# jkomijani/normflow_

Hardware: AMD Instinct MI355X
Metric: lattice configs/sec (forward+logdet) (higher is better)
Workload: dtype f32

## Files before the change

### normflow__amd/_hip.py

```python
import ctypes as C
import os
import threading
import weakref

import torch

_HERE = os.path.dirname(os.path.abspath(__file__))
LIB_PATH = os.path.join(_HERE, "lib", "libnormflow_hip.so")

NF_F32, NF_F64, NF_F16, NF_F16_FIELD = 0, 1, 2, 3
LAYOUT_FULL, LAYOUT_PAIR = 0, 1
EXTRAP = {None: 0, 'none': 0, 'linear': 1, 'anti': 2, 'anti-periodic': 2}


OPT_SPLIT16, OPT_PIPE, OPT_SMALL8 = 0, 1, 2


class NormflowHipError(RuntimeError):
    pass


class RqsOpts(C.Structure):
    _fields_ = [("m", C.c_int32), ("extrap_left", C.c_int32), ("extrap_right", C.c_int32),
                ("layout", C.c_int32), ("xlo", C.c_double), ("xhi", C.c_double),
# ... 528 lines not shown
    return wp.reshape(nt, 16, cin_pad // 4, 4, ntaps).permute(4, 2, 0, 3, 1).contiguous()


def conv_weight_for_layer(w, lat4, k4, cin, cout, compact, fused, dtype_code):
    frag = pack_conv_weight(w)
    code = load().nf_conv_weight_layout(lat4, k4, cin, cout, int(compact), int(fused), dtype_code)
    if code < 0:
        raise RuntimeError("nf_conv_weight_layout: invalid layer description")
    if code == 0:
        return frag
    if code == 2:
        return pack_conv_weight_split16(w)
    ntaps, kq, nt = frag.shape[:3]
    k3 = w.shape[-1]
    rows = ntaps // k3
    vals = frag.reshape(rows, k3, kq, nt, 64).permute(0, 2, 4, 1, 3).reshape(rows, kq, 64, k3 * nt)
    nv = (k3 * nt + 3) // 4 * 4
    out = vals.new_zeros(rows, kq, 64, nv)
    out[..., :k3 * nt] = vals
    return out.contiguous()


SPLIT16_WEIGHT_SCALE = 1024.0


def pack_conv_weight_split16(w):
    cout, cin = w.shape[:2]
    assert cin == 8 and tuple(w.shape[2:]) == (3, 3, 3, 3) and cout <= 48
    wp = w.new_zeros(48, 8, 28, 3, dtype=torch.float32)
    wp[:cout, :, :27] = w.reshape(cout, 8, 27, 3).float() * SPLIT16_WEIGHT_SCALE
    hi = wp.half()
    lo = (wp - hi.float()).half()
    out = torch.empty(3, 21, 2, 64, 8, dtype=torch.float16, device=w.device)
    for k, part in enumerate((hi, lo)):
        v = part.reshape(3, 16, 8, 7, 4, 3).permute(0, 5, 3, 4, 1, 2)
        out[:, :, k] = v.reshape(3, 21, 64, 8)
    return out.contiguous()


def pack_conv_weight_split16_two_site(w):
    assert tuple(w.shape) == (8, 8, 3, 3, 3, 3)
    wr = w.reshape(8, 8, 27, 3).float() * SPLIT16_WEIGHT_SCALE
    w2 = wr.new_zeros(16, 8, 27, 4)
    w2[:8, :, :, :3] = wr
    w2[8:, :, :, 1:] = wr
    hi = w2.half()
    lo = (w2 - hi.float()).half()
    out = torch.empty(27, 2, 64, 8, dtype=torch.float16, device=w.device)
    for k, part in enumerate((hi, lo)):
        out[:, k] = part.permute(2, 3, 0, 1).reshape(27, 64, 8)
    return out.contiguous()


def pack_conv_weight_split16_first(w):
    assert tuple(w.shape) == (8, 1, 3, 3, 3, 3)
    wr = w.reshape(8, 27, 3).float() * SPLIT16_WEIGHT_SCALE
    w2 = wr.new_zeros(16, 32, 4)
    w2[:8, :27, :3] = wr
    w2[8:, :27, 1:] = wr
    hi = w2.half()
    lo = (w2 - hi.float()).half()
    out = torch.empty(4, 2, 64, 8, dtype=torch.float16, device=w.device)
    for k, part in enumerate((hi, lo)):
        v = part.reshape(16, 4, 4, 2, 4).permute(1, 2, 0, 3, 4)
        out[:, k] = v.reshape(4, 64, 8)
    return out.contiguous()


def conv_first_split16(x, weight, bias, act, weight_src=None):
    lib = load()
    B = x.shape[0]
    lat = list(x.shape[2:])
    lat4 = (C.c_int32 * 4)(*lat)
    V = 1
    for n in lat:
        V *= n
    wsp = _cached_pack(weight if weight_src is None else weight_src, 'first16', pack_conv_weight_split16_first)
    bias = None if bias is None else bias.detach().float().contiguous()
    out = torch.empty((B, V, 16), dtype=torch.float16, device=x.device)
    step = max(1, min(MAX_B, ((1 << 31) - 1) // V))
    for b0 in range(0, B, step):
        b1 = min(B, b0 + step)
        _check(lib.nf_conv_first_split16(_ptr(x[b0:b1]), _ptr(wsp), _ptr(bias), _ptr(out[b0:b1]), b1 - b0, lat4,
                                         int(act), _stream()), "nf_conv_first_split16")
    return out


def _split16_site_index(L3, device):
    slot = torch.arange(L3 // 2, device=device)
    return torch.stack((2 * slot, (2 * slot - 1) % L3))


def to_split16(h):
    B, Cc = h.shape[:2]
    L3 = h.shape[-1]
    if Cc != 8 or L3 % 2:
        raise NormflowHipError("to_split16: 8 channels and an even fastest axis expected")
    hp = h.reshape(B, 8, -1, L3).float()
    idx = _split16_site_index(L3, h.device)
    g = hp[..., idx].permute(0, 2, 3, 4, 1)
    hi = g.half()
    lo = (g - hi.float()).half()
    return torch.stack((hi, lo), dim=2).reshape(B, -1, 16).contiguous()


def from_split16(h16, lattice):
    B = h16.shape[0]
    L3 = lattice[-1]
    t = h16.reshape(B, -1, 2, 2, L3 // 2, 8).float()
    v = t[:, :, 0] + t[:, :, 1]
    idx = _split16_site_index(L3, h16.device)
    out = torch.empty((B, v.shape[1], L3, 8), dtype=torch.float32, device=h16.device)
    out[:, :, idx.reshape(-1)] = v.reshape(B, v.shape[1], L3, 8)
    return out.permute(0, 3, 1, 2).reshape((B, 8) + tuple(lattice)).contiguous()


def conv_layer_split16(h16, weight, bias, act, lattice):
    lib = load()
    B = h16.shape[0]
    lat4 = (C.c_int32 * 4)(*lattice)
    wsp = _cached_pack(weight, 'two_site16', pack_conv_weight_split16_two_site)
    bias = None if bias is None else bias.detach().float().contiguous()
    out = torch.empty_like(h16)
    for b0 in range(0, B, MAX_B):
        b1 = min(B, b0 + MAX_B)
        _check(lib.nf_conv_fwd_split16(_ptr(h16[b0:b1]), _ptr(wsp), _ptr(bias), _ptr(out[b0:b1]), b1 - b0, lat4,
                                       int(act), _stream()), "nf_conv_fwd_split16")
    return out


_UNIT_OK = {}


def invalidate_weight_checks():
    _UNIT_OK.clear()
    _PACKED.clear()


_PACKED = {}
_PACK_IN_CAPTURE = [False]


class pack_inside_capture:

    def __enter__(self):
        self._old = _PACK_IN_CAPTURE[0]
        _PACK_IN_CAPTURE[0] = True

    def __exit__(self, *exc):
        _PACK_IN_CAPTURE[0] = self._old
        return False


def _cached_pack(w, kind, fn):
    if _PACK_IN_CAPTURE[0] and torch.cuda.is_current_stream_capturing():
        return fn(w.detach())
    base = w._base if w._base is not None else w
    key = (id(base), kind)
    state = (w._version, w.data_ptr(), tuple(w.shape), w.dtype)
    hit = _PACKED.get(key)
    if hit is not None and hit[0]() is base and hit[1] == state:
        return hit[2]
    out = fn(w.detach())
    _PACKED[key] = (weakref.ref(base, lambda _, k=key: _PACKED.pop(k, None)), state, out)
    return out


def _weights_fit_fp16(w):
    base = w._base if w._base is not None else w
    key = id(base)
    state = (w._version, w.data_ptr(), tuple(w.shape))
    hit = _UNIT_OK.get(key)
    if hit is not None and hit[0]() is base and hit[1] == state:
        return hit[2]
# ... 120 lines not shown
            if split:
                need = lib.nf_conv_wgrad_split16_workspace(b1 - b0, lat4, cin)
                ws = torch.empty(int(need), dtype=torch.uint8, device=x.device)
                if bits is None:
                    bits = absmax_bits(gz)
                _check(lib.nf_conv_wgrad_split16(_ptr(x[b0:b1]), _ptr(part[b0:b1]), _ptr(buf), b1 - b0, lat4, k4, cin,
                                                 c1 - c0, _ptr(bits), int(compact_parity), _ptr(ws), ws.numel(), _stream()),
                       "nf_conv_wgrad_split16")
            elif sites:
                need = lib.nf_conv_wgrad_sites_workspace(k4, cin, c1 - c0, _dtype_code(x))
                ws = torch.empty(int(need), dtype=torch.uint8, device=x.device)
                _check(lib.nf_conv_wgrad_sites(_ptr(x[b0:b1]), _ptr(part[b0:b1]), _ptr(buf), b1 - b0, lat4, k4, cin,
                                               c1 - c0, int(compact_parity), _ptr(ws), ws.numel(), _dtype_code(x), _stream()),
                       "nf_conv_wgrad_sites")
            else:
                _check(lib.nf_conv_wgrad(_ptr(x[b0:b1]), _ptr(part[b0:b1]), _ptr(buf), b1 - b0, lat4, k4, cin,
                                         c1 - c0, _dtype_code(x), _stream()), "nf_conv_wgrad")
        gws.append(buf[:c1 - c0, :ntaps * cin])
        gbs.append(buf[:c1 - c0, ntaps * cin])
    gw = torch.cat(gws) if len(gws) > 1 else gws[0]
    gb = torch.cat(gbs) if len(gbs) > 1 else gbs[0]
    gw = gw.reshape(cout, ntaps, cin).permute(0, 2, 1).reshape((cout, cin) + tuple(ksize))
    return gw, gb


def conv_input_grad_split16(gz, wt, bits=None, compact_parity=-1, lattice=None, weight=None):
    lib = load()
    cin = wt.shape[0]
    if compact_parity < 0:
        lattice = tuple(gz.shape[2:])
    if (gz.dtype != torch.float32 or lattice is None or len(lattice) != 4 or cin > 8 or tuple(wt.shape[2:]) != (3, 3, 3, 3)
            or not lib.nf_get_option(OPT_SPLIT16)):
        return None
    B, Cc = gz.shape[:2]
    lat4, k4 = _lat4(lattice, (3, 3, 3, 3))
    if not lib.nf_conv_split16_supported(lat4, k4, 8, 8, ACT_CODES['tanh']) or B > 65535:
        return None
    if not _weights_fit_fp16(wt if weight is None else weight):
        return None
    G = (Cc + 7) // 8
    V = 1
    for n in lattice:
        V *= n
    gz = gz.contiguous()
    g16 = torch.empty((G, B, V, 16), dtype=torch.float16, device=gz.device)
    if bits is None:
        bits = absmax_bits(gz)
    _check(lib.nf_planes_to_split16(_ptr(gz), _ptr(g16), _ptr(bits), B, Cc, lat4, int(compact_parity), _stream()),
           "nf_planes_to_split16")
    gx = torch.empty((B, 8) + tuple(lattice), dtype=torch.float32, device=gz.device)
    wpad = wt.new_zeros((8, 8 * G, 3, 3, 3, 3), dtype=torch.float32)
    wpad[:cin, :Cc] = wt.float()
    for g in range(G):
        wsp = pack_conv_weight_split16_two_site(wpad[:, 8 * g:8 * g + 8].contiguous())
        _check(lib.nf_conv_dgrad_split16(_ptr(g16[g]), _ptr(wsp), None, _ptr(gx), B, lat4, _ptr(bits), int(g > 0), 0,
                                         _stream()), "nf_conv_dgrad_split16")
    return gx if cin == 8 else gx[:, :cin].contiguous()


def conv_hidden_planes_split16(x, weight, bias, act):
    lib = load()
    if (x.dtype != torch.float32 or x.dim() != 6 or tuple(weight.shape) != (8, 8, 3, 3, 3, 3) or act not in (0, ACT_CODES['tanh'])
            or not lib.nf_get_option(OPT_SPLIT16)):
        return None
    B = x.shape[0]
    lattice = tuple(x.shape[2:])
    lat4, k4 = _lat4(lattice, (3, 3, 3, 3))
    if not lib.nf_conv_split16_supported(lat4, k4, 8, 8, ACT_CODES['tanh']) or B > 65535 or not _weights_fit_fp16(weight):
        return None
    V = x[0, 0].numel()
    x16 = torch.empty((1, B, V, 16), dtype=torch.float16, device=x.device)
    bits = absmax_bits(x)
    _check(lib.nf_planes_to_split16(_ptr(x), _ptr(x16), _ptr(bits), B, 8, lat4, -1, _stream()), "nf_planes_to_split16")
    wsp = pack_conv_weight_split16_two_site(weight.detach().float())
    out = torch.empty_like(x)
    b = None if bias is None else bias.detach().float().contiguous()
    _check(lib.nf_conv_dgrad_split16(_ptr(x16[0]), _ptr(wsp), _ptr(b), _ptr(out), B, lat4, _ptr(bits), 0, int(act), _stream()),
           "nf_conv_dgrad_split16")
    return out


def conv_last_logits_split16(x, weight, bias, parity):
    lib = load()
    if (x.dtype != torch.float32 or x.dim() != 6 or tuple(weight.shape) != (46, 8, 3, 3, 3, 3) or x.shape[1] != 8
            or x.shape[-1] < 32 or x.shape[-1] % 16 or any(n < 2 or n % 2 for n in x.shape[2:5])
            or not lib.nf_get_option(OPT_SPLIT16) or not _weights_fit_fp16(weight)):
        return None
    B = x.shape[0]
    lattice = tuple(x.shape[2:])
    lat4 = (C.c_int32 * 4)(*lattice)
    V = x[0, 0].numel()
    bits = absmax_bits(x)
    wsp = pack_conv_weight_split16(weight.detach().float())
    b = None if bias is None else bias.detach().float().contiguous()
    out = torch.empty((B, 46, V // 2), dtype=torch.float32, device=x.device)
    src, is16 = x, 0
    if lattice[-1] != 32:
        src = torch.empty((1, B, V, 16), dtype=torch.float16, device=x.device)
        _check(lib.nf_planes_to_split16(_ptr(x), _ptr(src), _ptr(bits), B, 8, lat4, -1, _stream()), "nf_planes_to_split16")
        is16 = 1
    _check(lib.nf_conv_last_logits_split16(_ptr(src), is16, _ptr(wsp), _ptr(b), _ptr(out), B, lat4, int(parity), _ptr(bits),
                                           _stream()), "nf_conv_last_logits_split16")
    return out


def pack_wide_split16(w1, b1, w2, b2, w3, b3):
    h, cout = w1.shape[0], w3.shape[0]
    f = lambda t: t.detach().float()
    w1p = f(w1).new_zeros((16, 1, 3, 3, 3, 3)); w1p[:h] = f(w1)
    w2p = f(w2).new_zeros((16, 16, 3, 3, 3, 3)); w2p[:h, :h] = f(w2)
    w3p = f(w3).new_zeros((cout, 16, 3, 3, 3, 3)); w3p[:, :h] = f(w3)
    padb = lambda b, n: None if b is None else torch.nn.functional.pad(f(b), (0, n - b.shape[0]))
    b1p, b2p = padb(b1, 16), padb(b2, 16)
    cut = lambda b, g: None if b is None else b[8 * g:8 * g + 8].contiguous()
    first = [(pack_conv_weight_split16_first(w1p[8 * g:8 * g + 8].contiguous()), cut(b1p, g)) for g in (0, 1)]
    hidden = [[pack_conv_weight_split16_two_site(w2p[8 * go:8 * go + 8, 8 * gi:8 * gi + 8].contiguous()) for gi in (0, 1)] for go in (0, 1)]
    last = [pack_conv_weight_split16(w3p[:, 8 * gi:8 * gi + 8].contiguous()) for gi in (0, 1)]
    return first, (hidden, [cut(b2p, 0), cut(b2p, 1)]), (last, None if b3 is None else f(b3).contiguous()), cout


def conv_wide_logits_split16(x, packed, act1, parity):
    lib = load()
    first, (hidden, hb), (last, b3), cout = packed
    B = x.shape[0]
    lattice = tuple(x.shape[2:])
    lat4 = (C.c_int32 * 4)(*lattice)
    V = x[0, 0].numel()
    x = x.contiguous()
    tanh = ACT_CODES['tanh']
    h1 = []
    for wsp, b in first:
        out = torch.empty((B, V, 16), dtype=torch.float16, device=x.device)
        _check(lib.nf_conv_first_split16(_ptr(x), _ptr(wsp), _ptr(b), _ptr(out), B, lat4, int(act1), _stream()), "nf_conv_first_split16")
        h1.append(out)
    h2 = []
    z = torch.empty((B, 8) + lattice, dtype=torch.float32, device=x.device)
    for go in (0, 1):
        for gi in (0, 1):
            _check(lib.nf_conv_dgrad_split16(_ptr(h1[gi]), _ptr(hidden[go][gi]), _ptr(hb[go]) if gi == 0 else None, _ptr(z), B, lat4, None,
                                             int(gi > 0), tanh if gi == 1 else 0, _stream()), "nf_conv_dgrad_split16")
        out = torch.empty((1, B, V, 16), dtype=torch.float16, device=x.device)
        _check(lib.nf_planes_to_split16(_ptr(z), _ptr(out), None, B, 8, lat4, -1, _stream()), "nf_planes_to_split16")
        h2.append(out)
    del h1
    logits = torch.empty((B, cout, V // 2), dtype=torch.float32, device=x.device)
    for gi in (0, 1):
        _check(lib.nf_conv_last_logits_split16_acc(_ptr(h2[gi]), 1, _ptr(last[gi]), _ptr(b3) if gi == 0 else None, _ptr(logits), B, lat4,
                                                   int(parity), None, int(gi > 0), int(cout), _stream()), "nf_conv_last_logits_split16_acc")
    return logits


class ConvFn(torch.autograd.Function):

    @staticmethod
    def forward(ctx, x, weight, bias, act, compact, parity):
        _require_device(x, weight, bias)
        x = x.contiguous()
        out = None
        if not compact and x.dim() == 6 and x.shape[1] == 8 and weight.shape[0] == 8:
            out = conv_hidden_planes_split16(x, weight, bias, act)
        elif compact and act == 0 and x.dim() == 6 and weight.shape[0] == 46:
            out = conv_last_logits_split16(x, weight, bias, parity)
        if out is None:
            out = _conv_launch(x, weight.detach(), bias, act, compact, parity, weight_src=weight)
        ctx.save_for_backward(x, weight, out if act else None)
        ctx.act, ctx.compact, ctx.parity, ctx.has_bias = act, compact, parity, bias is not None
        return out

    @staticmethod
# ... 81 lines not shown
        return y, logj

    @staticmethod
    def backward(ctx, gy, glogj):
        h, weight, bias, xpt = ctx.saved_tensors
        lib = load()
        B, V = xpt.shape
        lattice = tuple(h.shape[2:])
        lat4 = (C.c_int32 * 4)(*lattice)
        cout = weight.shape[0]
        bits = absmax_bits(h)
        src, is16 = FusedLastRqsFn._source(h, bits, lat4)
        wsp = pack_conv_weight_split16(weight.detach().float())
        b = None if bias is None else bias.detach().float().contiguous()
        gz = torch.empty((B, cout, V // 2), dtype=torch.float32, device=h.device)
        gx = torch.empty_like(xpt)
        _check(lib.nf_conv_rqs_split16_vjp(_ptr(src), is16, _ptr(wsp), _ptr(b), cout, _ptr(xpt), _ptr(gy.contiguous()),
                                           _ptr(glogj.contiguous()), _ptr(gz), _ptr(gx), B, lat4, int(ctx.parity), _ptr(bits),
                                           C.byref(ctx.opts), int(bool(ctx.inverse)), _stream()), "nf_conv_rqs_split16_vjp")
        gh = gw = gb = None
        gbits = absmax_bits(gz)
        if ctx.needs_input_grad[0]:
            wt = weight.detach().flip([2, 3, 4, 5]).transpose(0, 1).contiguous()
            gh = conv_input_grad_split16(gz, wt, gbits, ctx.parity, lattice, weight)
        if ctx.needs_input_grad[1] or (bias is not None and ctx.needs_input_grad[2]):
            got = conv_weight_grad(h, gz, weight.shape[2:], gbits, ctx.parity)
            if got is not None:
                gw, gb = got
        if (ctx.needs_input_grad[0] and gh is None) or ((ctx.needs_input_grad[1] or ctx.needs_input_grad[2]) and gw is None):
            raise NormflowHipError("FusedLastRqsFn.backward: the split-fp16 gradient kernels refused a layer the forward pass took")
        if bias is None:
            gb = None
        return gh, gw, gb, gx, (glogj if ctx.has_log0 else None), None, None, None


def conv_layer(x, weight, bias, act=0, compact=False, parity=0):
    if torch.is_grad_enabled() and (x.requires_grad or weight.requires_grad or (bias is not None and bias.requires_grad)):
        if act == 5:
            return torch.abs(ConvFn.apply(x, weight, bias, 0, compact, parity))
        return ConvFn.apply(x, weight, bias, act, compact, parity)
    x = x.contiguous()
    return _conv_launch(x, weight.detach(), None if bias is None else bias.detach(), act, compact, parity, weight_src=weight)


def conv_affine_split16(h16, weight, bias, x_active, log0, parity, inverse, lattice, out=None):
    _require_device(h16, weight, bias, x_active, log0)
    lib = load()
    B, V = x_active.shape
    x_active = x_active.contiguous()
    lat4 = (C.c_int32 * 4)(*lattice)
    def pack_affine(w):
        w8 = w.new_zeros((8, 8, 3, 3, 3, 3), dtype=torch.float32)
        w8[:2] = w.float()
        return pack_conv_weight_split16_two_site(w8)
    wsp = _cached_pack(weight, 'affine16', pack_affine)
    b8 = torch.zeros(8, dtype=torch.float32, device=x_active.device)
    if bias is not None:
        b8[:2] = bias.detach().float()
    field16 = x_active.dtype == torch.float16
    if out is None:
        y = torch.empty_like(x_active)
        logj = torch.empty(B, dtype=torch.float32, device=x_active.device)
    else:
        y, logj = out
    ws = _workspace(min(B, MAX_B), V, x_active.device)
    for b0 in range(0, B, MAX_B):
        b1 = min(B, b0 + MAX_B)
        l0 = log0[b0:b1] if log0 is not None else None
        _check(lib.nf_conv_affine_split16(_ptr(h16[b0:b1]), _ptr(wsp), _ptr(b8), _ptr(x_active[b0:b1]), _ptr(l0),
                                          _ptr(y[b0:b1]), _ptr(logj[b0:b1]), b1 - b0, lat4, int(parity), int(inverse),
                                          4 if field16 else 0, _ptr(ws), ws.numel(), _stream()), "nf_conv_affine_split16")
    return y, logj


def conv_rqs(h, weight, bias, x_active, log0, parity, opts, inverse, unit_input=False, lattice=None, out=None):
    _require_device(h, weight, bias, x_active, log0)
    lib = load()
    h, x_active = h.contiguous(), x_active.contiguous()
    split_in = lattice is not None
    B = h.shape[0]
    cin = weight.shape[1] if split_in else h.shape[1]
    lat = list(lattice) if split_in else list(h.shape[2:])
    d = len(lat)
    lat4 = (C.c_int32 * 4)(*([1] * (4 - d) + lat))
    k4 = (C.c_int32 * 4)(*([1] * (4 - d) + list(weight.shape[2:])))
    V = x_active.shape[1]
    flags = 1 if (unit_input and _weights_fit_fp16(weight)) else 0
    field16 = x_active.dtype == torch.float16
    if field16:
        flags |= 4
    ldt = torch.float32 if field16 else x_active.dtype
    if split_in:
        if not flags or h.dtype != torch.float16 or tuple(h.shape) != (B, V, 16):
            raise NormflowHipError("split-fp16 hidden activations need unit_input and a (B, V, 16) half tensor")
        flags |= 2
    fused_code = 1 | ((flags & 1) << 1) | ((flags & 2) << 1)
    kind = ('fused_last', tuple(lat4), tuple(k4), cin, fused_code, lib.nf_get_option(OPT_SPLIT16), lib.nf_get_option(OPT_PIPE))
    wfrag = _cached_pack(weight, kind, lambda w: conv_weight_for_layer(w, lat4, k4, cin, w.shape[0], True, fused_code, NF_F32))
    bias = None if bias is None else bias.detach().contiguous()
    if out is None:
        y = torch.empty_like(x_active)
        logj = torch.empty(B, dtype=ldt, device=x_active.device)
    else:
        y, logj = out
        if (tuple(y.shape) != (B, V) or tuple(logj.shape) != (B,) or y.dtype != x_active.dtype or logj.dtype != ldt
                or not y.is_contiguous() or not logj.is_contiguous()):
            raise NormflowHipError("conv_rqs: `out` must be contiguous (B, V) and (B,) tensors of the input's dtype (log|J| fp32 for a half field)")
        _require_device(y, logj)
# ... 157 lines not shown
```

### normflow__amd/csrc/nf_conv_g.hip

```cpp
#include <hip/hip_runtime.h>
#include <hip/hip_fp16.h>
#include "nf_conv_core.h"

namespace nf {

typedef _Float16 f16x8 __attribute__((ext_vector_type(8)));
typedef _Float16 f16x4 __attribute__((ext_vector_type(4)));

#if !defined(NF_DIAG) || !defined(NF_G2_ABL)
#undef NF_G2_ABL
#define NF_G2_ABL 0
#endif

namespace g2 {
template <bool SEGM>
struct Geo {
  static constexpr int RBL = SEGM ? 1088 : 1024;
  static constexpr int PLROWS = 16;
  static constexpr int PLANE = PLROWS * RBL;
  static constexpr int NSLOT = 8;
  static constexpr int RING = NSLOT * PLANE;
  static constexpr int XBUF = 4 * 2 * 64 * 16;
  static constexpr int LDS_BYTES = RING + 2 * XBUF;
  static_assert(LDS_BYTES <= 160 * 1024, "ring + exchange must fit the CU's LDS");
};
#ifndef NF_G2_PRIO
#define NF_G2_PRIO 1
#endif
constexpr int NSA = 14;
constexpr float kInvWScale = 1.0f / 1024.0f;
}

__device__ __forceinline__ float tanh_affine(float a, float c1, float c0) {
  const float t = __builtin_amdgcn_exp2f(__builtin_fmaf(a, c1, c0));
  return __builtin_fmaf(-2.0f, __builtin_amdgcn_rcpf(1.0f + t), 1.0f);
}
__device__ __forceinline__ float act_affine(float a, float c1, float c0, float al, float ga) {
  const float t = __builtin_amdgcn_exp2f(__builtin_fmaf(a, c1, c0));
  return __builtin_fmaf(al, __builtin_amdgcn_rcpf(1.0f + t), ga);
}

template <bool SEGM, int EPI, bool HK = false>
__global__ __launch_bounds__(512, 2) void conv_g2_kernel(ConvArgs A) {
  using namespace g2;
  typedef Geo<SEGM> G;
  constexpr int RBL = G::RBL, PLANE = G::PLANE, NSLOT = G::NSLOT, RING = G::RING, XBUF = G::XBUF;
  extern __shared__ __align__(16) unsigned char smem_g2[];
  const int lane = threadIdx.x & 63;
  const int wave = __builtin_amdgcn_readfirstlane(threadIdx.x >> 6);
  const bool isB = wave >= 4;
  const int q = wave & 3;
  const int g = lane >> 4, p = lane & 15;
  const unsigned lds0 = unsigned(reinterpret_cast<size_t>((__attribute__((address_space(3))) unsigned char *)smem_g2));

  const int n0 = A.L[0] >> 1, n1 = A.L[1] >> 1, ncol = n0 * n1;
  const int L2 = A.L[2], nstep = L2 >> 1;
  const int L3 = A.L[3], HP = L3 >> 1, NSEG = (HP + 15) >> 4;
  const int RB = L3 * 32, HB = L3 * 16, PB = L3 * 8;
  const int seg_lo = SEGM ? A.seg_lo : 0, seg_n = SEGM ? (A.seg_n > 0 ? A.seg_n : NSEG) : 1;
  const int total = int(A.nitems);
  const int xcd = blockIdx.x & 7, jm = blockIdx.x >> 3;
  auto col_id = [&](int ci) { return (xcd + 8 * ci) * 32 + jm; };
  int ncols_my = 0;
  {
    const int first = col_id(0);
    if (first < total) ncols_my = (total - first + 255) / 256;
  }
  if (ncols_my == 0) return;
  const int td0 = NSEG == 1 ? 1 : ((n0 & 3) == 0 ? 4 : ((n0 & 1) == 0 ? 2 : 1));
  const int td1 = NSEG == 1 ? 1 : ((n1 & 3) == 0 ? 4 : ((n1 & 1) == 0 ? 2 : 1));
  auto decode = [&](int ci, int &b, int &i0, int &i1, int &hs) {
    int gc = col_id(ci);
    hs = 0;
    if (SEGM) {
      hs = seg_lo + gc % seg_n;
      gc /= seg_n;
    }
    b = gc / ncol;
    int c = gc - b * ncol;
    const int t1 = c % td1; c /= td1;
    const int t0 = c % td0; c /= td0;
    const int nt1 = n1 / td1;
    i0 = (c / nt1) * td0 + t0;
    i1 = (c % nt1) * td1 + t1;
  };

  const int sl0 = isB ? NSA : 0;
  f16x8 bh[NSA], bl[NSA];
  {
    const f16x8 *__restrict__ wsp = static_cast<const f16x8 *>(A.wfrag) + lane;
#pragma unroll
    for (int r = 0; r < NSA; ++r) {
      const int rr = sl0 + r;
      const int rc = rr < 27 ? rr : 26;
      bh[r] = wsp[(2 * rc) * 64];
      bl[r] = wsp[(2 * rc + 1) * 64];
    }
  }
  float bv4[4], kc0[4];
#pragma unroll
  for (int r = 0; r < 4; ++r) {
    bv4[r] = A.bias ? static_cast<const float *>(A.bias)[4 * (g & 1) + r] : 0.f;
  }
  const bool is_tanh = A.act != kActSigmoid;
  const float kcs = is_tanh ? 2.885390081777927f : -1.4426950408889634f;
  const float kal = is_tanh ? -2.0f : 1.0f, kga = is_tanh ? 1.0f : 0.0f;
#pragma unroll
  for (int r = 0; r < 4; ++r) kc0[r] = kcs * bv4[r];
  const float kc1 = kcs * kInvWScale;
  [[maybe_unused]] const float descale = kInvWScale / pow2_scale_for(A.gscale_bits);

  const int ja = p + (g >> 1), para = (g + 1) & 1;
  const unsigned rowsel = unsigned(((q >> 1) * 4 + (q & 1)) * RBL);
  const unsigned lane_a = rowsel + unsigned((SEGM && ja == 16) ? 1024 + para * 16 : para * 256 + (ja & 15) * 16);
  const unsigned lane_al = lane_a + unsigned((SEGM && ja == 16) ? 32 : 512);
  constexpr bool HALF = SEGM && EPI != 3 && HK;
  const int psh = p >> 3, pm = p & 7;
  const int lane_am_delta = int(rowsel + unsigned(para * 256 + (pm + (g >> 1)) * 16)) - int(lane_a);
  const int hz0 = wave >> 1, hz1a = 2 * (wave & 1);
  unsigned lane_d = unsigned(lane * 16), lane_d2 = 0;
  const unsigned char *__restrict__ inb = static_cast<const unsigned char *>(A.in);
  const int64_t sampleB = A.V * 32;

  int ici = 0, ipl = -1, head = 0;
  const unsigned char *rowp[2] = {nullptr, nullptr};
  auto open_issue_column = [&]() {
    int ib, ii0, ii1, hs;
    decode(ici, ib, ii0, ii1, hs);
    int x0 = 2 * ii0 + hz0 - 1;
    x0 = x0 < 0 ? x0 + A.L[0] : (x0 >= A.L[0] ? x0 - A.L[0] : x0);
#pragma unroll
    for (int k = 0; k < 2; ++k) {
      int x1 = 2 * ii1 + hz1a + k - 1;
      x1 = x1 < 0 ? x1 + A.L[1] : (x1 >= A.L[1] ? x1 - A.L[1] : x1);
      rowp[k] = inb + int64_t(ib) * sampleB + int64_t((x0 * A.L[1] + x1) * L2) * RB;
    }
    if (SEGM) {
      const int blk = lane >> 4;
      int gs = 16 * hs + (lane & 15);
      gs = gs >= HP ? gs - HP : gs;
      lane_d = unsigned((blk >> 1) * HB + (blk & 1) * PB + gs * 16);
      int g17 = 16 * hs + 16;
      g17 = g17 >= HP ? g17 - HP : g17;
      lane_d2 = unsigned(((lane >> 1) & 1) * HB + (lane & 1) * PB + g17 * 16);
    }
  };
  open_issue_column();
  const unsigned lds_rows = lds0 + unsigned((hz0 * 4 + hz1a) * RBL);
  constexpr int PPP = SEGM ? 2 : 1;
  auto issue_piece = [&](int k) {
    if (ici >= ncols_my) return false;
    const int x2 = ipl < 0 ? L2 - 1 : (ipl >= L2 ? 0 : ipl);
    const unsigned char *src = rowp[k] + unsigned(x2) * unsigned(RB);
    const unsigned dst = lds_rows + unsigned((head & (NSLOT - 1)) * PLANE + k * RBL);
    dma_row(src, lane_d, dst);
    if (SEGM) {
      if (lane < 4) dma_row(src, lane_d2, dst + 1024u);
    }
    if (k == 1) {
      ++head;
      if (++ipl > L2) {
        ipl = -1;
        if (++ici < ncols_my) open_issue_column();
      }
    }
    return true;
  };
  auto issue_entry = [&]() { return issue_piece(0) && issue_piece(1); };

#pragma unroll 1
  for (int e = 0; e < NSLOT; ++e) (void)issue_entry();
// ... 80 lines not shown
        hi[r] = h0;
        lo[r] = static_cast<_Float16>(v - static_cast<float>(h0));
      }
      if (plane_ok) {
        unsigned char *d = pout + plane_o;
        *reinterpret_cast<f16x4 *>(d) = hi;
        *reinterpret_cast<f16x4 *>(d + HB) = lo;
      }
    } else if constexpr (EPI == 3) {
      if (plane_ok) {
        float *d = static_cast<float *>(A.out) + pfield + int64_t(4 * (g & 1)) * A.V;
#pragma unroll
        for (int r = 0; r < 4; ++r) {
          float v = (prev[r] + pa[r]) * descale + bv4[r];
          if (A.accumulate) v += pold[r];
          if (A.act == kActTanh) v = tanh_affine(v, 2.885390081777927f, 0.f);
          d[int64_t(r) * A.V] = v;
        }
      }
    } else {
      if (pslot != aslot) {
        flush();
        aslot = pslot;
      }
      if (plane_ok) {
        const float t = (prev[0] + pa[0]) * kInvWScale + bv4[0];
        const float sa = __builtin_fabsf((prev[1] + pa[1]) * kInvWScale + bv4[1]);
        const float2 xv = load_field_pair(A, pfield);
        const int a = g >> 1;
        const float v = a ? xv.y : xv.x;
        const float val = EPI == 2 ? (v - t) * nf_exp(sa) : t + v * nf_exp(-sa);
        float2 ov;
        ov.x = a ? 0.f : val;
        ov.y = a ? val : 0.f;
        store_field_pair(A, pfield, ov);
        lacc += double(EPI == 2 ? sa : -sa);
      }
    }
  };

  for (int k = 0; k < nsteps_total; ++k) {
    int ndma = 0;
    if (EPI == 3 && A.accumulate) {
      if (lane_ok) {
        const float *d = static_cast<const float *>(A.out) + fcol + int64_t(2 * s) * L3 + int64_t(4 * (g & 1)) * A.V;
#pragma unroll
        for (int r = 0; r < 4; ++r) nold[r] = d[int64_t(r) * A.V];
      }
    }
    if (!(NF_G2_ABL & 1) && free_next == 4) {
      ndma += issue_entry() ? 2 * PPP : 0;
      ndma += issue_entry() ? 2 * PPP : 0;
    }
    const bool refill = !(NF_G2_ABL & 1) && free_next >= 2;
    auto dma_slot = [&](int i) {
      if (refill && issue_piece(i & 1)) ndma += PPP;
    };
    NF_G2TICK(0)
    if (isB && have_prev && !(NF_G2_ABL & 2)) epilogue((k - 1) & 1);
    NF_G2TICK(1)
#if NF_G2_PRIO
    __builtin_amdgcn_s_setprio(2);
#endif
    f32x4 am[2], ac[2];
    am[0] = am[1] = ac[0] = ac[1] = f32x4{0.f, 0.f, 0.f, 0.f};
    unsigned rowa[4], rowl[4];
#pragma unroll
    for (int i = 0; i < 4; ++i) {
      const unsigned po = unsigned(((rbase + i) & (NSLOT - 1)) * PLANE);
      rowa[i] = po + lane_a;
      rowl[i] = po + lane_al;
    }
    auto fetch = [&](f16x8 (&fh)[4], f16x8 (&fl)[4], int coff, int I0, int I1, int H0, int H1) {
      if constexpr (HALF) {
#pragma unroll
        for (int i = 0; i < 3; ++i) {
          if (i < H0 || i > H1) continue;
          const unsigned rm = unsigned(((rbase + i + psh) & (NSLOT - 1)) * PLANE) + unsigned(int(lane_a) + lane_am_delta);
          fh[i] = *reinterpret_cast<const f16x8 *>(smem_g2 + rm + coff);
          fl[i] = *reinterpret_cast<const f16x8 *>(smem_g2 + rm + 512 + coff);
        }
        return;
      }
#pragma unroll
      for (int i = 0; i < 4; ++i) {
        if (i < I0 || i > I1) continue;
        if (NF_G2_ABL & 8) {
          fh[i] = bh[i]; fl[i] = bl[i];
          asm volatile("" : "+v"(fh[i]), "+v"(fl[i]));
        } else {
          fh[i] = *reinterpret_cast<const f16x8 *>(smem_g2 + rowa[i] + coff);
          fl[i] = *reinterpret_cast<const f16x8 *>(smem_g2 + rowl[i] + coff);
        }
      }
    };
    auto mult = [&](const f16x8 (&fh)[4], const f16x8 (&fl)[4], int base, int J0, int J1) {
      if (NF_G2_ABL & 4) {
#pragma unroll
        for (int i = 0; i < 4; ++i) asm volatile("" ::"v"(fh[i]), "v"(fl[i]));
        return;
      }
      if constexpr (HALF) {
#pragma unroll
        for (int j2 = 0; j2 < 3; ++j2)
          if (j2 >= J0 && j2 <= J1) am[0] = __builtin_amdgcn_mfma_f32_16x16x32_f16(bh[base + j2], fh[j2], am[0], 0, 0, 0);
#pragma unroll
        for (int j2 = 0; j2 < 3; ++j2)
          if (j2 >= J0 && j2 <= J1) ac[0] = __builtin_amdgcn_mfma_f32_16x16x32_f16(bl[base + j2], fh[j2], ac[0], 0, 0, 0);
#pragma unroll
        for (int j2 = 0; j2 < 3; ++j2)
          if (j2 >= J0 && j2 <= J1) ac[0] = __builtin_amdgcn_mfma_f32_16x16x32_f16(bh[base + j2], fl[j2], ac[0], 0, 0, 0);
        return;
      }
#pragma unroll
      for (int j2 = 0; j2 < 3; ++j2)
#pragma unroll
        for (int t = 0; t < 2; ++t)
          if (j2 >= J0 && j2 <= J1) am[t] = __builtin_amdgcn_mfma_f32_16x16x32_f16(bh[base + j2], fh[t + j2], am[t], 0, 0, 0);
#pragma unroll
      for (int j2 = 0; j2 < 3; ++j2)
#pragma unroll
        for (int t = 0; t < 2; ++t)
          if (j2 >= J0 && j2 <= J1) ac[t] = __builtin_amdgcn_mfma_f32_16x16x32_f16(bl[base + j2], fh[t + j2], ac[t], 0, 0, 0);
#pragma unroll
      for (int j2 = 0; j2 < 3; ++j2)
#pragma unroll
        for (int t = 0; t < 2; ++t)
          if (j2 >= J0 && j2 <= J1) ac[t] = __builtin_amdgcn_mfma_f32_16x16x32_f16(bh[base + j2], fl[t + j2], ac[t], 0, 0, 0);
    };
    auto combo_off = [](int jj) { return ((jj / 3) * 4 + jj % 3) * RBL; };
    f16x8 fh0[4], fl0[4], fh1[4], fl1[4];
#define NF_SB __builtin_amdgcn_sched_barrier(0)
    if (!isB) {
      fetch(fh0, fl0, combo_off(0), 0, 3, 0, 2);
      fetch(fh1, fl1, combo_off(1), 0, 3, 0, 2);
      NF_SB; mult(fh0, fl0, 0, 0, 2); NF_SB;
      dma_slot(0);
      fetch(fh0, fl0, combo_off(2), 0, 3, 0, 2);
      NF_SB; mult(fh1, fl1, 3, 0, 2); NF_SB;
      dma_slot(1);
      fetch(fh1, fl1, combo_off(3), 0, 3, 0, 2);
      NF_SB; mult(fh0, fl0, 6, 0, 2); NF_SB;
      dma_slot(2);
      fetch(fh0, fl0, combo_off(4), 0, 2, 0, 1);
      NF_SB; mult(fh1, fl1, 9, 0, 2); NF_SB;
      dma_slot(3);
      mult(fh0, fl0, 12, 0, 1);
      NF_SB;
    } else {
      fetch(fh0, fl0, combo_off(4), 2, 3, 2, 2);
      fetch(fh1, fl1, combo_off(5), 0, 3, 0, 2);
      NF_SB; mult(fh0, fl0, 12 - NSA, 2, 2); NF_SB;
      fetch(fh0, fl0, combo_off(6), 0, 3, 0, 2);
      NF_SB; mult(fh1, fl1, 15 - NSA, 0, 2); NF_SB;
      dma_slot(0);
      fetch(fh1, fl1, combo_off(7), 0, 3, 0, 2);
      NF_SB; mult(fh0, fl0, 18 - NSA, 0, 2); NF_SB;
      dma_slot(1);
      fetch(fh0, fl0, combo_off(8), 0, 3, 0, 2);
      NF_SB; mult(fh1, fl1, 21 - NSA, 0, 2); NF_SB;
      dma_slot(2);
      mult(fh0, fl0, 24 - NSA, 0, 2);
      NF_SB;
      dma_slot(3);
    }
#undef NF_SB
#if NF_G2_PRIO
    __builtin_amdgcn_s_setprio(0);
#endif
    if (!isB && have_prev && !(NF_G2_ABL & 2)) epilogue((k - 1) & 1);
    NF_G2TICK(2)
#pragma unroll
    for (int t = 0; t < 2; ++t)
#pragma unroll
      for (int r = 0; r < 4; ++r) am[t][r] += ac[t][r];
    constexpr bool mh = HALF;
    *reinterpret_cast<f32x4 *>(smem_g2 + (k & 1) * XBUF + xsend) = (isB || mh) ? am[0] : am[1];
    prev = (isB && !mh) ? am[1] : am[0];
    pout = ocol + unsigned(2 * s) * unsigned(RB);
    plane_o = lane_o;
    plane_ok = lane_ok;
    if (EPI == 3) {
      pfield = fcol + int64_t(2 * s) * L3;
      pold = nold;
    } else if (EPI > 0) {
      pfield = fcol + int64_t(2 * s) * HP;
      pslot = col_slot;
    }
    have_prev = true;
    const int allow = s + 1 == nstep ? 0 : ndma;
    if (allow >= 16) wait_vm<16>();
    else if (allow >= 12) wait_vm<12>();
    else if (allow >= 8) wait_vm<8>();
    else if (allow >= 6) wait_vm<6>();
    else if (allow >= 4) wait_vm<4>();
    else if (allow >= 2) wait_vm<2>();
    else wait_vm<0>();
    NF_G2TICK(3)
    lds_barrier();
    NF_G2TICK(4)
    if (++s == nstep) {
      s = 0;
      free_next = 4;
      rbase += 4;
      if (++cci < ncols_my) open_column(cci);
    } else {
      free_next = 2;
      rbase += 2;
    }
  }
#if defined(NF_DIAG) && defined(NF_G2_TIMING)
  if (blockIdx.x == 9 && lane == 0 && (wave == 0 || wave == 4) && nsteps_total > 100)
    printf("[g2 timing] wave %d steps %d | cycles per step: head %.0f  epilogue %.0f  mfma %.0f  wait %.0f  barrier %.0f\n", wave, nsteps_total,
           double(tacc[0]) / nsteps_total, double(tacc[1]) / nsteps_total, double(tacc[2]) / nsteps_total, double(tacc[3]) / nsteps_total, double(tacc[4]) / nsteps_total);
#endif
  if (have_prev) epilogue((nsteps_total - 1) & 1);
  if (EPI == 1 || EPI == 2) flush();
  wait_vm<0>();
}

}

using namespace nf;

extern "C" int nf_conv_split16_supported(const int32_t *lattice, const int32_t *ksize, int cin, int cout, int act) {
  if (!nf::option(NF_OPT_SPLIT16) || !lattice || !ksize || cin != 8 || cout != 8) return 0;
  if (act != kActTanh && act != kActSigmoid) return 0;
  for (int mu = 0; mu < 4; ++mu)
    if (ksize[mu] != 3) return 0;
  if (lattice[3] < 32 || (lattice[3] & 15)) return 0;
  for (int mu = 0; mu < 3; ++mu)
    if (lattice[mu] < 2 || (lattice[mu] & 1)) return 0;
  return 1;
}

static int launch_g2(ConvArgs &A, const int32_t *lattice, int64_t B, int epi, hipStream_t stream, const char *what) {
  A.V = 1;
  for (int mu = 0; mu < 4; ++mu) {
    A.L[mu] = lattice[mu]; A.k[mu] = 3;
    A.V *= lattice[mu];
  }
  A.cin = 8; A.cout = 8;
  const bool segm = lattice[3] != 32;
// ... 104 lines not shown
```

Measured before the change: 961.6.

## Restructure split16 conv MFMA schedule with stacked hi/lo weight packing

Measured after the change: 979.6, median of 6. 1.9% higher.

```diff
diff --git a/normflow__amd/_hip.py b/normflow__amd/_hip.py
--- a/normflow__amd/_hip.py
+++ b/normflow__amd/_hip.py
@@ -604,6 +604,17 @@
     return out.contiguous()
 
 
+def pack_conv_weight_split16_stacked(w):
+    assert tuple(w.shape) == (8, 8, 3, 3, 3, 3)
+    wr = w.reshape(8, 8, 9, 3, 3).float() * SPLIT16_WEIGHT_SCALE
+    hi = wr.half()
+    lo = (wr - hi.float()).half()
+    parts = torch.stack((hi, lo))[:, :, :, :8]
+    v = parts.reshape(2, 8, 8, 2, 4, 3, 3).permute(3, 5, 6, 4, 0, 1, 2)
+    stacked = v.reshape(18, 64, 8)
+    return torch.cat((stacked, pack_conv_weight_split16_two_site(w).reshape(54, 64, 8))).contiguous()
+
+
 def pack_conv_weight_split16_first(w):
     assert tuple(w.shape) == (8, 1, 3, 3, 3, 3)
     wr = w.reshape(8, 27, 3).float() * SPLIT16_WEIGHT_SCALE
@@ -671,7 +682,7 @@
     lib = load()
     B = h16.shape[0]
     lat4 = (C.c_int32 * 4)(*lattice)
-    wsp = _cached_pack(weight, 'two_site16', pack_conv_weight_split16_two_site)
+    wsp = _cached_pack(weight, 'stacked16', pack_conv_weight_split16_stacked)
     bias = None if bias is None else bias.detach().float().contiguous()
     out = torch.empty_like(h16)
     for b0 in range(0, B, MAX_B):
@@ -898,7 +909,7 @@
     wpad = wt.new_zeros((8, 8 * G, 3, 3, 3, 3), dtype=torch.float32)
     wpad[:cin, :Cc] = wt.float()
     for g in range(G):
-        wsp = pack_conv_weight_split16_two_site(wpad[:, 8 * g:8 * g + 8].contiguous())
+        wsp = pack_conv_weight_split16_stacked(wpad[:, 8 * g:8 * g + 8].contiguous())
         _check(lib.nf_conv_dgrad_split16(_ptr(g16[g]), _ptr(wsp), None, _ptr(gx), B, lat4, _ptr(bits), int(g > 0), 0,
                                          _stream()), "nf_conv_dgrad_split16")
     return gx if cin == 8 else gx[:, :cin].contiguous()
@@ -918,7 +929,7 @@
     x16 = torch.empty((1, B, V, 16), dtype=torch.float16, device=x.device)
     bits = absmax_bits(x)
     _check(lib.nf_planes_to_split16(_ptr(x), _ptr(x16), _ptr(bits), B, 8, lat4, -1, _stream()), "nf_planes_to_split16")
-    wsp = pack_conv_weight_split16_two_site(weight.detach().float())
+    wsp = pack_conv_weight_split16_stacked(weight.detach().float())
     out = torch.empty_like(x)
     b = None if bias is None else bias.detach().float().contiguous()
     _check(lib.nf_conv_dgrad_split16(_ptr(x16[0]), _ptr(wsp), _ptr(b), _ptr(out), B, lat4, _ptr(bits), 0, int(act), _stream()),
@@ -960,7 +971,7 @@
     b1p, b2p = padb(b1, 16), padb(b2, 16)
     cut = lambda b, g: None if b is None else b[8 * g:8 * g + 8].contiguous()
     first = [(pack_conv_weight_split16_first(w1p[8 * g:8 * g + 8].contiguous()), cut(b1p, g)) for g in (0, 1)]
-    hidden = [[pack_conv_weight_split16_two_site(w2p[8 * go:8 * go + 8, 8 * gi:8 * gi + 8].contiguous()) for gi in (0, 1)] for go in (0, 1)]
+    hidden = [[pack_conv_weight_split16_stacked(w2p[8 * go:8 * go + 8, 8 * gi:8 * gi + 8].contiguous()) for gi in (0, 1)] for go in (0, 1)]
     last = [pack_conv_weight_split16(w3p[:, 8 * gi:8 * gi + 8].contiguous()) for gi in (0, 1)]
     return first, (hidden, [cut(b2p, 0), cut(b2p, 1)]), (last, None if b3 is None else f(b3).contiguous()), cout
 
@@ -1148,8 +1159,8 @@
     def pack_affine(w):
         w8 = w.new_zeros((8, 8, 3, 3, 3, 3), dtype=torch.float32)
         w8[:2] = w.float()
-        return pack_conv_weight_split16_two_site(w8)
-    wsp = _cached_pack(weight, 'affine16', pack_affine)
+        return pack_conv_weight_split16_stacked(w8)
+    wsp = _cached_pack(weight, 'affine16s', pack_affine)
     b8 = torch.zeros(8, dtype=torch.float32, device=x_active.device)
     if bias is not None:
         b8[:2] = bias.detach().float()
diff --git a/normflow__amd/csrc/nf_conv_g.hip b/normflow__amd/csrc/nf_conv_g.hip
--- a/normflow__amd/csrc/nf_conv_g.hip
+++ b/normflow__amd/csrc/nf_conv_g.hip
@@ -27,7 +27,6 @@
 #ifndef NF_G2_PRIO
 #define NF_G2_PRIO 1
 #endif
-constexpr int NSA = 14;
 constexpr float kInvWScale = 1.0f / 1024.0f;
 }
 
@@ -85,16 +84,17 @@
     i1 = (c % nt1) * td1 + t1;
   };
 
-  const int sl0 = isB ? NSA : 0;
-  f16x8 bh[NSA], bl[NSA];
+  f16x8 wp[9], bt[15];
   {
     const f16x8 *__restrict__ wsp = static_cast<const f16x8 *>(A.wfrag) + lane;
 #pragma unroll
-    for (int r = 0; r < NSA; ++r) {
-      const int rr = sl0 + r;
-      const int rc = rr < 27 ? rr : 26;
-      bh[r] = wsp[(2 * rc) * 64];
-      bl[r] = wsp[(2 * rc + 1) * 64];
+    for (int r = 0; r < 9; ++r) wp[r] = wsp[((isB ? 9 : 0) + r) * 64];
+#pragma unroll
+    for (int r = 0; r < 15; ++r) {
+      constexpr int kSP = 18;
+      const int fa = r < 12 ? 2 * (3 * (r < 9 ? r / 3 : 8) + r % 3) : 2 * (24 + r - 12) + 1;
+      const int fb = 2 * (3 * (r < 9 ? 5 + r / 3 : 3 + (r - 9) / 3) + r % 3);
+      bt[r] = wsp[(kSP + (isB ? fb : fa)) * 64];
     }
   }
   float bv4[4], kc0[4];
@@ -117,6 +117,16 @@
   constexpr bool HALF = SEGM && EPI != 3 && HK;
   const int psh = p >> 3, pm = p & 7;
   const int lane_am_delta = int(rowsel + unsigned(para * 256 + (pm + (g >> 1)) * 16)) - int(lane_a);
+  unsigned lane_p[4];
+  {
+    const int cP = (isB ? 4 : 0) + g;
+    const unsigned coffP = unsigned(((cP / 3) * 4 + cP % 3) * RBL);
+#pragma unroll
+    for (int xp = 0; xp < 4; ++xp) {
+      const int jx = (HALF ? pm : p) + (xp >> 1), parx = (xp + 1) & 1;
+      lane_p[xp] = rowsel + coffP + unsigned((SEGM && jx == 16) ? 1024 + parx * 16 : parx * 256 + (jx & 15) * 16);
+    }
+  }
   const int hz0 = wave >> 1, hz1a = 2 * (wave & 1);
   unsigned lane_d = unsigned(lane * 16), lane_d2 = 0;
   const unsigned char *__restrict__ inb = static_cast<const unsigned char *>(A.in);
@@ -303,6 +313,7 @@
       ndma += issue_entry() ? 2 * PPP : 0;
       ndma += issue_entry() ? 2 * PPP : 0;
     }
+    const int ndma_head = ndma;
     const bool refill = !(NF_G2_ABL & 1) && free_next >= 2;
     auto dma_slot = [&](int i) {
       if (refill && issue_piece(i & 1)) ndma += PPP;
@@ -314,7 +325,8 @@
     __builtin_amdgcn_s_setprio(2);
 #endif
     f32x4 am[2], ac[2];
-    am[0] = am[1] = ac[0] = ac[1] = f32x4{0.f, 0.f, 0.f, 0.f};
+    f32x4 pe[2], po[2];
+    if (NF_G2_ABL & 4) pe[0] = pe[1] = po[0] = po[1] = f32x4{0.f, 0.f, 0.f, 0.f};
     unsigned rowa[4], rowl[4];
 #pragma unroll
     for (int i = 0; i < 4; ++i) {
@@ -322,99 +334,117 @@
       rowa[i] = po + lane_a;
       rowl[i] = po + lane_al;
     }
-    auto fetch = [&](f16x8 (&fh)[4], f16x8 (&fl)[4], int coff, int I0, int I1, int H0, int H1) {
+    auto fetch = [&](f16x8 (&f)[4], int coff, bool lo) {
       if constexpr (HALF) {
 #pragma unroll
         for (int i = 0; i < 3; ++i) {
-          if (i < H0 || i > H1) continue;
           const unsigned rm = unsigned(((rbase + i + psh) & (NSLOT - 1)) * PLANE) + unsigned(int(lane_a) + lane_am_delta);
-          fh[i] = *reinterpret_cast<const f16x8 *>(smem_g2 + rm + coff);
-          fl[i] = *reinterpret_cast<const f16x8 *>(smem_g2 + rm + 512 + coff);
+          f[i] = *reinterpret_cast<const f16x8 *>(smem_g2 + rm + (lo ? 512 : 0) + coff);
         }
         return;
       }
 #pragma unroll
       for (int i = 0; i < 4; ++i) {
-        if (i < I0 || i > I1) continue;
         if (NF_G2_ABL & 8) {
-          fh[i] = bh[i]; fl[i] = bl[i];
-          asm volatile("" : "+v"(fh[i]), "+v"(fl[i]));
+          f[i] = bt[i];
+          asm volatile("" : "+v"(f[i]));
         } else {
-          fh[i] = *reinterpret_cast<const f16x8 *>(smem_g2 + rowa[i] + coff);
-          fl[i] = *reinterpret_cast<const f16x8 *>(smem_g2 + rowl[i] + coff);
+          f[i] = *reinterpret_cast<const f16x8 *>(smem_g2 + (lo ? rowl[i] : rowa[i]) + coff);
         }
       }
     };
-    auto mult = [&](const f16x8 (&fh)[4], const f16x8 (&fl)[4], int base, int J0, int J1) {
-      if (NF_G2_ABL & 4) {
-#pragma unroll
-        for (int i = 0; i < 4; ++i) asm volatile("" ::"v"(fh[i]), "v"(fl[i]));
-        return;
-      }
-      if constexpr (HALF) {
-#pragma unroll
-        for (int j2 = 0; j2 < 3; ++j2)
-          if (j2 >= J0 && j2 <= J1) am[0] = __builtin_amdgcn_mfma_f32_16x16x32_f16(bh[base + j2], fh[j2], am[0], 0, 0, 0);
-#pragma unroll
-        for (int j2 = 0; j2 < 3; ++j2)
-          if (j2 >= J0 && j2 <= J1) ac[0] = __builtin_amdgcn_mfma_f32_16x16x32_f16(bl[base + j2], fh[j2], ac[0], 0, 0, 0);
-#pragma unroll
-        for (int j2 = 0; j2 < 3; ++j2)
-          if (j2 >= J0 && j2 <= J1) ac[0] = __builtin_amdgcn_mfma_f32_16x16x32_f16(bh[base + j2], fl[j2], ac[0], 0, 0, 0);
-        return;
-      }
+    auto fetch_p = [&](f16x8 (&f)[4], int i) {
+      if (HALF && i > 2) return;
+      const unsigned pl = unsigned(((rbase + i + (HALF ? psh : 0)) & (NSLOT - 1)) * PLANE);
+#pragma unroll
+      for (int xp = 0; xp < 4; ++xp) {
+        if (NF_G2_ABL & 8) {
+          f[xp] = bt[xp];
+          asm volatile("" : "+v"(f[xp]));
+        } else {
+          f[xp] = *reinterpret_cast<const f16x8 *>(smem_g2 + pl + lane_p[xp]);
+        }
+      }
+    };
+    auto consume = [](const f16x8 (&f)[4]) {
+#pragma unroll
+      for (int i = 0; i < 4; ++i) asm volatile("" ::"v"(f[i]));
+    };
+    auto mult_p = [&](const f16x8 (&f)[4], int i) {
+      if (NF_G2_ABL & 4) return consume(f);
+#pragma unroll
+      for (int dx = 0; dx < 3; ++dx)
+#pragma unroll
+        for (int t = 0; t < 2; ++t) {
+          const int j2 = i - t;
+          if (j2 < 0 || j2 > 2 || (HALF && t > 0)) continue;
+          const bool first = j2 == 0 && dx == 0;
+          pe[t] = __builtin_amdgcn_mfma_f32_16x16x32_f16(wp[3 * j2 + dx], f[dx], first ? f32x4{0.f, 0.f, 0.f, 0.f} : pe[t], 0, 0, 0);
+          po[t] = __builtin_amdgcn_mfma_f32_16x16x32_f16(wp[3 * j2 + dx], f[dx + 1], first ? f32x4{0.f, 0.f, 0.f, 0.f} : po[t], 0, 0, 0);
+        }
+    };
+    constexpr int NT = HALF ? 1 : 2;
+    auto mult_q = [&](const f16x8 (&fl)[4], int hb) {
+      if (NF_G2_ABL & 4) return consume(fl);
 #pragma unroll
       for (int j2 = 0; j2 < 3; ++j2)
 #pragma unroll
-        for (int t = 0; t < 2; ++t)
-          if (j2 >= J0 && j2 <= J1) am[t] = __builtin_amdgcn_mfma_f32_16x16x32_f16(bh[base + j2], fh[t + j2], am[t], 0, 0, 0);
+        for (int t = 0; t < NT; ++t) ac[t] = __builtin_amdgcn_mfma_f32_16x16x32_f16(bt[hb + j2], fl[t + j2], ac[t], 0, 0, 0);
+    };
+    auto mult_hh = [&](const f16x8 (&fh)[4], int hb) {
+      if (NF_G2_ABL & 4) return;
 #pragma unroll
       for (int j2 = 0; j2 < 3; ++j2)
 #pragma unroll
-        for (int t = 0; t < 2; ++t)
-          if (j2 >= J0 && j2 <= J1) ac[t] = __builtin_amdgcn_mfma_f32_16x16x32_f16(bl[base + j2], fh[t + j2], ac[t], 0, 0, 0);
-#pragma unroll
-      for (int j2 = 0; j2 < 3; ++j2)
-#pragma unroll
-        for (int t = 0; t < 2; ++t)
-          if (j2 >= J0 && j2 <= J1) ac[t] = __builtin_amdgcn_mfma_f32_16x16x32_f16(bh[base + j2], fl[t + j2], ac[t], 0, 0, 0);
+        for (int t = 0; t < NT; ++t) am[t] = __builtin_amdgcn_mfma_f32_16x16x32_f16(bt[hb + j2], fh[t + j2], am[t], 0, 0, 0);
+    };
+    auto combine = [&]() {
+#pragma unroll
+      for (int t = 0; t < 2; ++t)
+#pragma unroll
+        for (int r = 0; r < 4; ++r) {
+          const auto sw = __builtin_amdgcn_permlane32_swap(__float_as_uint(pe[t][r]), __float_as_uint(po[t][r]), false, false);
+          am[t][r] = __uint_as_float(sw[0]);
+          ac[t][r] = __uint_as_float(sw[1]);
+        }
     };
     auto combo_off = [](int jj) { return ((jj / 3) * 4 + jj % 3) * RBL; };
-    f16x8 fh0[4], fl0[4], fh1[4], fl1[4];
+    f16x8 u0[4], u1[4], v0[4], v1[4];
 #define NF_SB __builtin_amdgcn_sched_barrier(0)
+    fetch_p(u0, 0);
+    fetch_p(u1, 1);
+    fetch_p(v0, 2);
+    fetch_p(v1, 3);
+    NF_SB; mult_p(u0, 0); mult_p(u1, 1); NF_SB;
+    dma_slot(0);
     if (!isB) {
-      fetch(fh0, fl0, combo_off(0), 0, 3, 0, 2);
-      fetch(fh1, fl1, combo_off(1), 0, 3, 0, 2);
-      NF_SB; mult(fh0, fl0, 0, 0, 2); NF_SB;
-      dma_slot(0);
-      fetch(fh0, fl0, combo_off(2), 0, 3, 0, 2);
-      NF_SB; mult(fh1, fl1, 3, 0, 2); NF_SB;
-      dma_slot(1);
-      fetch(fh1, fl1, combo_off(3), 0, 3, 0, 2);
-      NF_SB; mult(fh0, fl0, 6, 0, 2); NF_SB;
-      dma_slot(2);
-      fetch(fh0, fl0, combo_off(4), 0, 2, 0, 1);
-      NF_SB; mult(fh1, fl1, 9, 0, 2); NF_SB;
-      dma_slot(3);
-      mult(fh0, fl0, 12, 0, 1);
+      fetch(u0, combo_off(8), true);
+      fetch(u1, combo_off(8), false);
+    } else {
+      fetch(u0, combo_off(3), true);
+      fetch(u1, combo_off(4), true);
+    }
+    NF_SB; mult_p(v0, 2); mult_p(v1, 3); NF_SB;
+    dma_slot(1);
+    if (!isB) {
+      fetch(v0, combo_off(0), true);
+      fetch(v1, combo_off(1), true);
+    } else {
+      fetch(v0, combo_off(5), true);
+      fetch(v1, combo_off(6), true);
+    }
+    combine();
+    NF_SB; mult_q(u0, 9); mult_q(u1, 12); NF_SB;
+    if (!isB) {
+      mult_hh(u1, 9);
       NF_SB;
-    } else {
-      fetch(fh0, fl0, combo_off(4), 2, 3, 2, 2);
-      fetch(fh1, fl1, combo_off(5), 0, 3, 0, 2);
-      NF_SB; mult(fh0, fl0, 12 - NSA, 2, 2); NF_SB;
-      fetch(fh0, fl0, combo_off(6), 0, 3, 0, 2);
-      NF_SB; mult(fh1, fl1, 15 - NSA, 0, 2); NF_SB;
-      dma_slot(0);
-      fetch(fh1, fl1, combo_off(7), 0, 3, 0, 2);
-      NF_SB; mult(fh0, fl0, 18 - NSA, 0, 2); NF_SB;
-      dma_slot(1);
-      fetch(fh0, fl0, combo_off(8), 0, 3, 0, 2);
-      NF_SB; mult(fh1, fl1, 21 - NSA, 0, 2); NF_SB;
-      dma_slot(2);
-      mult(fh0, fl0, 24 - NSA, 0, 2);
-      NF_SB;
-      dma_slot(3);
-    }
+    }
+    dma_slot(2);
+    fetch(u0, combo_off(isB ? 7 : 2), true);
+    NF_SB; mult_q(v0, 0); mult_q(v1, 3); NF_SB;
+    dma_slot(3);
+    mult_q(u0, 6);
+    NF_SB;
 #undef NF_SB
 #if NF_G2_PRIO
     __builtin_amdgcn_s_setprio(0);
@@ -439,7 +469,7 @@
       pslot = col_slot;
     }
     have_prev = true;
-    const int allow = s + 1 == nstep ? 0 : ndma;
+    const int allow = s + 1 == nstep ? 0 : ndma - ndma_head;
     if (allow >= 16) wait_vm<16>();
     else if (allow >= 12) wait_vm<12>();
     else if (allow >= 8) wait_vm<8>();
```
